# laprade117/interactive-unet

Measured on AMD Instinct MI355X. Metric: voxels/sec (train step + full-volume predict) on 128^3 chunks, higher is better.
Workload: dtype bf16

## Files before the change

interactive-unet_amd/csrc/capi.hip:

```cpp
#include "common.h"
#include <cstdarg>
#include <cstdio>

static thread_local char g_err[512] = "";

void iunet_set_error(const char* fmt, ...) {
  va_list ap;
  va_start(ap, fmt);
  vsnprintf(g_err, sizeof(g_err), fmt, ap);
  va_end(ap);
}

#define DT_OK(dt) IUNET_REQUIRE((dt) == 0 || (dt) == 1, "dtype must be 0 (f16) or 1 (bf16), got %d", (dt))

extern "C" {

const char* iunet_last_error(void) { return g_err; }
int iunet_abi_version(void) { return 1; }

int iunet_conv3_num_tiles(int nd, int N, int D, int H, int W) { return iunet_conv3_tiles(nd, N, D, H, W); }

int iunet_conv3_stats_parts(int nd, int N, int D, int H, int W, int Cout, int layout) {
  return layout >= 2 ? iunet_conv3_v4_stats_parts(nd, Cout) : iunet_conv3_tiles(nd, N, D, H, W);
}

long long iunet_pack_conv3_elems(int Cout, int Cin, int taps, int mode) { return iunet_pack_conv3_size(Cout, Cin, taps, mode); }

int iunet_pack_conv3(int dtype, const void* w, const void* scale, void* dst, int Cout, int Cin, int taps, int mode,
                     void* stream) {
  DT_OK(dtype);
  IUNET_REQUIRE(w && dst, "pack_conv3: null pointer");
  IUNET_REQUIRE(taps == 9 || taps == 27, "pack_conv3: taps must be 9 or 27 (got %d)", taps);
  return iunet_pack_conv3_launch(dtype, (const float*)w, (const float*)scale, dst, Cout, Cin, taps, mode, (hipStream_t)stream);
}

int iunet_pack_first_conv(int dtype, const void* w, const void* scale, void* dst, int Cout, int Cin, int taps,
                          void* stream) {
  DT_OK(dtype);
  IUNET_REQUIRE(w && dst, "pack_first_conv: null pointer");
  IUNET_REQUIRE(Cout % 32 == 0 && Cin >= 1 && Cin <= 12, "pack_first_conv: Cout multiple of 32, Cin 1..4 (3..12: the virtual operator of iunet_x2_prep)");
  return iunet_pack_first_conv_launch(dtype, (const float*)w, (const float*)scale, dst, Cout, Cin, taps, (hipStream_t)stream);
}

long long iunet_pack_first_conv_elems(int Cout, int Cin, int taps) { return (long long)Cout * (((taps * Cin + 31) / 32) * 32); }

int iunet_pack_convT(int dtype, const void* w, void* dst, int Cin, int Cout, int npos, void* stream) {
  DT_OK(dtype);
  IUNET_REQUIRE(w && dst, "pack_convT: null pointer");
  IUNET_REQUIRE(npos == 4 || npos == 8, "pack_convT: npos must be 4 or 8");
  IUNET_REQUIRE(Cin % 32 == 0 && Cout % 32 == 0, "pack_convT: channels must be multiples of 32");
  return iunet_pack_convT_launch(dtype, (const float*)w, dst, Cin, Cout, npos, (hipStream_t)stream);
}

int iunet_conv3_pick_layout(int, int, int, int, int, int, int) { return 2; }

int iunet_conv3_compact_ok(int nd, int N, int D, int H, int W, int Cin, int Cout, int act, int bw) {
  if ((nd != 2 && nd != 3) || N < 1 || D < 1 || H < 1 || W < 1 || Cin < 32 || Cout < 32 || Cin % 32 || Cout % 32 || (bw && nd != 2)) return 0;
  if (nd == 2) return D == 1 && !((act || bw) && Cin > 64);
  if (Cin <= 32) return 0;
  return !(act && Cin > 192);
}

int iunet_conv3_packs_compact(int taps, int Cin) {
  IUNET_REQUIRE(taps == 9 || taps == 27, "conv3_packs_compact: taps must be 9 or 27 (got %d)", taps);
  IUNET_REQUIRE(Cin >= 32 && Cin % 32 == 0, "conv3_packs_compact: Cin must be a positive multiple of 32 (got %d)", Cin);
  return taps == 9 || Cin > 32;
}

int iunet_conv3_plan(int nd, int N, int D, int H, int W, int Cin, int Cout, int act, int bw, int have_compact, int* fused) {
  IUNET_REQUIRE(nd == 2 || nd == 3, "conv3_plan: nd must be 2 or 3 (got %d)", nd);
  IUNET_REQUIRE_GRID("conv3_plan", N, D, H, W);
  IUNET_REQUIRE(Cin >= 32 && Cout >= 32 && Cin % 32 == 0 && Cout % 32 == 0, "conv3_plan: channels must be positive multiples of 32 (%d, %d)", Cin, Cout);
  const int f = (act || bw) && (nd == 3 || Cin <= 64);
  if (fused) *fused = f;
  return have_compact && iunet_conv3_compact_ok(nd, N, D, H, W, Cin, Cout, act && f, bw && f) ? 3 : 2;
}

int iunet_conv3_tile_pairs(int nd, int N, int D, int H, int W, int Cin, int Cout) {
  if ((nd != 2 && nd != 3) || N < 1 || D < 1 || H < 1 || W < 1 || Cin < 32 || Cout < 32 || Cin % 32 || Cout % 32) return 0;
  return iunet_conv3_v4_pairs(nd, N, D, H, W, Cin, Cout, 0);
}

int iunet_conv3_fwd(int dtype, int nd, const void* x, long long x_sstride, void* y, long long y_sstride,
                    const void* wpk, const void* bias, void* stats, int N, int D, int H, int W, int Cin, int Cout,
                    int epi, int layout, void* stream) {
  DT_OK(dtype);
  IUNET_REQUIRE(x && y && wpk, "conv3: null pointer");
  IUNET_REQUIRE(N > 0 && D > 0 && H > 0 && W > 0, "conv3: bad shape %d %d %d %d", N, D, H, W);
  IUNET_REQUIRE(epi >= 0 && epi <= 2, "conv3: bad epilogue %d", epi);
  IUNET_REQUIRE(layout == 2 || layout == 3, "conv3: layout must be 2 or 3 (got %d)", layout);
  return iunet_conv3_launch(dtype, nd, x, x_sstride, y, y_sstride, wpk, (const float*)bias, (float*)stats, N, D, H, W,
                            Cin, Cout, epi, layout, (hipStream_t)stream);
}

int iunet_conv3_fwd_act(int dtype, int nd, const void* x, long long x_sstride, void* y, long long y_sstride,
                        const void* wpk, const void* bias, void* stats, const void* in_scale, const void* in_shift,
                        int N, int D, int H, int W, int Cin, int Cout, int epi, int layout, void* stream) {
  DT_OK(dtype);
  IUNET_REQUIRE(x && y && wpk && in_scale && in_shift, "conv3_act: null pointer");
  IUNET_REQUIRE(N > 0 && D > 0 && H > 0 && W > 0, "conv3: bad shape %d %d %d %d", N, D, H, W);
  IUNET_REQUIRE(epi >= 0 && epi <= 2, "conv3: bad epilogue %d", epi);
  IUNET_REQUIRE(layout == 2 || layout == 3, "conv3_act: the fused input activation exists in layouts 2 and 3 only (got %d)", layout);
  return iunet_conv3_launch(dtype, nd, x, x_sstride, y, y_sstride, wpk, (const float*)bias, (float*)stats, N, D, H, W,
                            Cin, Cout, epi, layout, (hipStream_t)stream, (const float*)in_scale, (const float*)in_shift);
}

int iunet_conv3_sample_stats_rows(int dtype, int nd, int N, int D, int H, int W, int Cin, int Cout, int layout) {
  DT_OK(dtype);
  if (layout < 2 || (nd != 2 && nd != 3) || N < 1 || D < 1 || H < 1 || W < 1 || Cin < 32 || Cout < 32 || Cin % 32 || Cout % 32) return 0;
  if (layout == 3 && !iunet_conv3_compact_ok(nd, N, D, H, W, Cin, Cout, 0, 0)) return 0;
  int rows = 0;
  if (iunet_conv3_v4_launch(dtype, nd, nullptr, 0, nullptr, 0, nullptr, nullptr, nullptr, N, D, H, W, Cin, Cout, 0, nullptr, nullptr, nullptr,
                            nullptr, 0, nullptr, layout == 3, 1, &rows) != IUNET_OK) return 0;
  return rows;
}

int iunet_conv3_fwd_sample_stats(int dtype, int nd, const void* x, long long x_sstride, void* y, long long y_sstride, const void* wpk,
                                 void* stats, int N, int D, int H, int W, int Cin, int Cout, int layout, void* stream) {
  DT_OK(dtype);
  IUNET_REQUIRE(x && y && wpk && stats, "conv3_fwd_sample_stats: null pointer");
  IUNET_REQUIRE_GRID("conv3_fwd_sample_stats", N, D, H, W);
  IUNET_REQUIRE(layout == 2 || layout == 3, "conv3_fwd_sample_stats: layout 2 or 3 (got %d)", layout);
  IUNET_REQUIRE(nd == 2 || nd == 3, "conv3: nd must be 2 or 3 (got %d)", nd);
  IUNET_REQUIRE(nd == 3 || D == 1, "conv3: 2-D conv needs D == 1");
  return iunet_conv3_v4_launch(dtype, nd, x, x_sstride, y, y_sstride, wpk, nullptr, (float*)stats, N, D, H, W, Cin, Cout, 0, nullptr, nullptr,
                               (hipStream_t)stream, nullptr, 0, nullptr, layout == 3, 1, nullptr);
}

int iunet_conv3_dgrad_sample_bnstats(int dtype, int nd, const void* dy, long long dy_sstride, void* dz, long long dz_sstride, const void* wpk,
// ... 209 lines not shown
```

interactive-unet_amd/csrc/conv3_v4.hip:

```cpp
#include "common.h"
#include <cstdlib>
#include <type_traits>

#ifdef IUNET_STAMPS
__device__ unsigned long long g_v4_stamps[4 * 512];
extern "C" int iunet_v4_stamps_read(unsigned long long* out) {
  return (int)hipMemcpyFromSymbol(out, HIP_SYMBOL(g_v4_stamps), sizeof(unsigned long long) * 4 * 512);
}
#endif
__device__ __attribute__((aligned(16))) unsigned int g_v4_zero16[4] = {0u, 0u, 0u, 0u};

namespace {

template <int ND, bool SMALL> struct V4Tile;
template <> struct V4Tile<3, false> { static constexpr int TZ = 4, TY = 8, TX = 16, PADZ = 1, NCOL = 9, S16 = 1, NCW = 8; };
template <> struct V4Tile<3, true>  { static constexpr int TZ = 2, TY = 8, TX = 16, PADZ = 1, NCOL = 9, S16 = 1, NCW = 4; };
template <bool SMALL> struct V4Tile<2, SMALL> { static constexpr int TZ = 1, TY = 16, TX = 32, PADZ = 0, NCOL = 3, S16 = 2, NCW = 8; };

#ifndef V4_BW_LT
#define V4_BW_LT 256
#endif
#ifndef V4_X2_LT3D
#define V4_X2_LT3D 512
#endif
#ifndef V4_RING2
#define V4_RING2 1
#endif
#ifndef V4_NP3_LT
#define V4_NP3_LT 512
#endif
constexpr int v4_loader_threads(int nd, bool ws, bool pair, bool spl, bool bwv = false, bool np = false) { return (ws || pair || ((spl || np) && nd == 2)) ? 256 : bwv ? V4_BW_LT : (spl && nd == 3) ? V4_X2_LT3D : (np && nd == 3) ? V4_NP3_LT : 512; }

struct ConvV4Params {
  const void* x;  long long x_sstride;
  void* y;        long long y_sstride;
  const void* wpk;
  const float* bias;
  const float* in_scale;
  const float* in_shift;
  float* stats;
  int N, D, H, W, Cin, Cout;
  int tilesZ, tilesY, tilesX;
  int bz, by, bx;
  int nbz, nby, nbx;
  int epi;
  int dbg;
  const void* bw_y; long long bw_y_ss;
  const float* bw_mean; const float* bw_invstd; const float* bw_scale; const float* bw_shift;
  int split_nc, x_lo, y_lo;
  const float* oscale;
  int* sat;
  int per_sample;
  int* query_rows;
};

template <typename T, int ND, bool WS, bool SMALL, bool BW = false, bool PAIR = false, bool NP = false, bool SPL = false>
__global__ __launch_bounds__((V4Tile<ND, SMALL>::NCW * 64 + v4_loader_threads(ND, WS, PAIR, SPL, BW, NP)), 1) void conv3_v4_kernel(ConvV4Params p) {
  static_assert(!SPL || (!WS && !BW && !PAIR && !(NP && ND == 3)), "split precision: streamed weights (Cin' = 3 Cin >= 96), forward only, padded operator in 3-D");
  static_assert(!PAIR || (!WS && !BW && ND == 3), "tile pairs: the streamed-weight 3-D forward / data-gradient variant only");
  static_assert(!NP || (!PAIR && (ND == 2 || !WS) && (!BW || (ND == 2 && WS))), "padding-free step: the streamed-weight 3-D variants and the 2-D ones; fused BatchNorm-backward sums on the 2-D resident-weights variant only");
  constexpr bool NP3 = NP && ND == 3, NP2 = NP && ND == 2;
  using V8 = typename Vec8<T>::type;
  using TL = V4Tile<ND, SMALL>;
  constexpr int NCW = TL::NCW, NLT = v4_loader_threads(ND, WS, PAIR, SPL, BW, NP);
  constexpr int TZ = TL::TZ, TY = TL::TY, TX = TL::TX, PADZ = TL::PADZ, NCOL = TL::NCOL, S16 = TL::S16;
  constexpr int FX = TX / 16, NI = TZ * TY * FX / NCW, NR = NI / FX;
  constexpr int PZ = TZ + 2 * PADZ, PY = TY + 2, PX = TX + 2;
  constexpr int NPIX = PZ * PY * PX;
  constexpr int PLANE = ((NPIX * 16 + 255) / 256) * 256;
  constexpr int CP = 2 * S16;
  constexpr int ABUF = CP * PLANE;
  constexpr int NCMB = (NCOL + 1) / 2, KS = NCMB * 3;
  constexpr int WBYTES = KS * 2 * 1024;
  constexpr int WSTEP = NP2 ? 3 * 3 * 2 * 1024 : S16 * WBYTES;
  constexpr bool RING2 = NP2 && !SPL && (WS ? (V4_RING2 & 1) != 0 : (V4_RING2 & 2) != 0);
  constexpr int NBUF = (NP3 || RING2) ? 3 : 2;
  constexpr int OFF_W = NBUF * ABUF;
  constexpr int WE = 4 * 3 * 2 * 1024, WO = WE + 3 * 2 * 1024;
  constexpr int AIT = (NPIX + NLT - 1) / NLT;
  constexpr int WIT = ((NP3 ? WO : WSTEP) / 16 + NLT - 1) / NLT;
  constexpr int NGRP = NP2 ? 3 : S16 * NCMB;
  constexpr int NRD = FX * (NR + 2) + 6;
  static_assert(NCW * NI == TZ * TY * FX, "consumer waves x fragments must cover the tile");

  extern __shared__ __attribute__((aligned(256))) unsigned char smem[];

  const int tid = threadIdx.x, lane = tid & 63;
  const int wave = __builtin_amdgcn_readfirstlane(tid >> 6);
  const int cob = blockIdx.y;
  const int nbricks = p.N * p.nbz * p.nby * p.nbx;
  const int bslots = p.bx * p.by * p.bz, ngrp = (int)gridDim.x / (8 * bslots);
  const int xcd = (blockIdx.x + (nbricks < 8 ? blockIdx.y : 0)) & 7, slot_all = blockIdx.x >> 3;
  const int grp = slot_all / bslots, slot = slot_all - grp * bslots;
  const int sx = slot % p.bx, sy = (slot / p.bx) % p.by, sz = slot / (p.bx * p.by);
  const int xb0 = (int)((long long)xcd * nbricks / 8), xb1 = (int)((long long)(xcd + 1) * nbricks / 8);
  const int b_begin = xb0 + (int)((long long)(xb1 - xb0) * grp / ngrp), b_end = xb0 + (int)((long long)(xb1 - xb0) * (grp + 1) / ngrp);
  const int nchunk = p.Cin / (16 * S16);
  const int nsteps = (b_end - b_begin) * nchunk;
  auto tile_of = [&](int s) -> int { return PAIR ? 2 * (s / (2 * nchunk)) + (s & 1) : s / nchunk; };
// ... 51 lines not shown
    }
    __syncthreads();
  }

  if (wave >= NCW) {
    const unsigned* zero16 = iunet_opaque_ptr((const unsigned*)g_v4_zero16);
    const int lt = tid - NCW * 64;
    int pcoord[AIT];
#pragma unroll
    for (int it = 0; it < AIT; ++it) {
      const int pix = min(lt + it * NLT, NPIX - 1);
      const int px = pix % PX, t2 = pix / PX;
      pcoord[it] = px | ((t2 % PY) << 8) | ((t2 / PY) << 16);
    }
    struct Staged { u32x4 a[AIT][CP]; unsigned ok; };
    const unsigned lds0 = (unsigned)(size_t)(__attribute__((address_space(3))) unsigned char*)smem;
    const int lw = __builtin_amdgcn_readfirstlane(lt >> 6);
    auto dma_weights = [&](int s, int buf, int it0 = 0, int it1 = 1 << 20) {
      const int chunk = chunk_of(s);
      const u32x4* ws = NP3 ? wsrc + (long long)(chunk >> 1) * ((WE + WO) / 16) + ((chunk & 1) ? WE / 16 : 0) : wsrc + (long long)chunk * (WSTEP / 16);
      const int nitem = NP3 ? ((chunk & 1) ? WO / 16 : WE / 16) : WSTEP / 16;
      const int woff = NP3 ? ((chunk & 1) ? WE : 0) : buf * WSTEP;
#pragma unroll
      for (int it = 0; it < WIT; ++it) {
        if (it < it0 || it >= it1) continue;
        const int base = it * NLT + lw * 64;
        if (base < nitem) {
          const u32x4* gsrc = ws + min(base + (lt & 63), nitem - 1);
          const unsigned dst = __builtin_amdgcn_readfirstlane(lds0 + OFF_W + woff + base * 16);
          unsigned keep;
          asm volatile("s_mov_b32 %0, m0\n\ts_mov_b32 m0, %2\n\ts_nop 0\n\tglobal_load_lds_dwordx4 %1, off\n\ts_mov_b32 m0, %0"
                       : "=&s"(keep) : "v"(gsrc), "s"(dst) : "memory");
        }
      }
    };
    auto load = [&](int s, Staged& r) {
      const int chunk = chunk_of(s);
      int n_img, z0, y0, x0;
      tile_origin(tile_of(s), n_img, z0, y0, x0);
      const T* xc = (const T*)p.x + (long long)n_img * p.x_sstride + src_plane(chunk) * plane_stride;
      r.ok = 0;
#pragma unroll
      for (int it = 0; it < AIT; ++it) {
        const int px = pcoord[it] & 255, py = (pcoord[it] >> 8) & 255, pz = pcoord[it] >> 16;
        const int gz = z0 + pz - PADZ, gy = y0 + py - 1, gx = x0 + px - 1;
        const bool ok = (unsigned)gz < (unsigned)p.D && (unsigned)gy < (unsigned)p.H && (unsigned)gx < (unsigned)p.W;
        const int cz = min(max(gz, 0), p.D - 1), cy = min(max(gy, 0), p.H - 1), cx = min(max(gx, 0), p.W - 1);
        const long long goff = (((long long)cz * p.H + cy) * p.W + cx) * 8;
#pragma unroll
        for (int k = 0; k < CP; ++k) r.a[it][k] = *(const u32x4*)(xc + k * plane_stride + goff);
        r.ok |= ok ? (1u << it) : 0u;
      }
    };
    auto dma_acts = [&](int s) {
      const int chunk = chunk_of(s);
      int n_img, z0, y0, x0;
      tile_origin(tile_of(s), n_img, z0, y0, x0);
      const T* xc = (const T*)p.x + (long long)n_img * p.x_sstride + src_plane(chunk) * plane_stride;
      const unsigned abuf = lds0 + abuf_of(s);
#pragma unroll
      for (int it = 0; it < AIT; ++it) {
        const int base = it * NLT + lw * 64;
        if (base < PLANE / 16) {
          const int pix = lt + it * NLT;
          const int px = pcoord[it] & 255, py = (pcoord[it] >> 8) & 255, pz = pcoord[it] >> 16;
          const int gz = z0 + pz - PADZ, gy = y0 + py - 1, gx = x0 + px - 1;
          const bool ok = pix < NPIX && (unsigned)gz < (unsigned)p.D && (unsigned)gy < (unsigned)p.H && (unsigned)gx < (unsigned)p.W;
          const long long goff = (((long long)gz * p.H + gy) * p.W + gx) * 8;
          if (pix < PLANE / 16) {
#pragma unroll
            for (int k = 0; k < CP; ++k) {
              const u32x4* gsrc = ok ? (const u32x4*)(xc + k * plane_stride + goff) : (const u32x4*)zero16;
              const unsigned dst = __builtin_amdgcn_readfirstlane(abuf + k * PLANE + base * 16);
              unsigned keep;
              asm volatile("s_mov_b32 %0, m0\n\ts_mov_b32 m0, %2\n\ts_nop 0\n\tglobal_load_lds_dwordx4 %1, off\n\ts_mov_b32 m0, %0"
                           : "=&s"(keep) : "v"(gsrc), "s"(dst) : "memory");
            }
          }
        }
      }
    };
    auto landed = [&]() { asm volatile("s_waitcnt vmcnt(0)" ::: "memory"); };
    auto commit = [&](int s, const Staged& r, auto ACT) {
      constexpr bool act = decltype(ACT)::value;
      unsigned char* ab = smem + abuf_of(s);
      const int cfirst = chunk_of(s) * CP * 8;
#pragma unroll
      for (int k = 0; k < CP; ++k) {
        float sc[8], sh[8];
        if (act) {
          const f32x4* ap = (const f32x4*)(smem + off_act) + (cfirst + k * 8) / 2;
          const f32x4 s0 = ap[0], s1 = ap[1], h0 = ap[2], h1 = ap[3];
#pragma unroll
          for (int j = 0; j < 4; ++j) { sc[j] = s0[j]; sc[4 + j] = s1[j]; sh[j] = h0[j]; sh[4 + j] = h1[j]; }
        }
#pragma unroll
        for (int it = 0; it < AIT; ++it) {
          const int pix = lt + it * NLT;
          u32x4 v = r.a[it][k];
          asm volatile("" : "+v"(v));
          if (pix < NPIX) {
            const bool ok = (r.ok >> it) & 1u;
            if (act) {
              const V8 in = __builtin_bit_cast(V8, v);
              V8 o;
#pragma unroll
              for (int j = 0; j < 8; ++j) o[j] = from_f32<T>(fmaxf(fmaf(sc[j], to_f32<T>(in[j]), sh[j]), 0.f));
              v = __builtin_bit_cast(u32x4, o);
            }
            *(u32x4*)(ab + k * PLANE + pix * 16) = ok ? v : u32x4{0u, 0u, 0u, 0u};
          }
        }
      }
    };
    auto run = [&](auto ACT) {
      const int last = nsteps - 1;
#ifdef V4_NOLOAD
      lds_barrier();
      for (int s = 0; s < nsteps; ++s) lds_barrier();
      return;
#endif
      if constexpr (RING2) if (!decltype(ACT)::value && !(p.dbg & 64)) {
        int K = 0;
#pragma unroll
        for (int it = 0; it < AIT; ++it) K += (it * NLT + lw * 64 < PLANE / 16) ? CP : 0;
        auto landed_but_last = [&]() {
          if (K == CP * AIT) asm volatile("s_waitcnt vmcnt(%0)" :: "i"(CP * AIT) : "memory");
          else if (K == CP * (AIT - 1)) asm volatile("s_waitcnt vmcnt(%0)" :: "i"(CP * (AIT - 1)) : "memory");
          else landed();
        };
        if (!WS) dma_weights(0, 0);
        dma_acts(0);
        if (last > 0) { dma_acts(1); landed_but_last(); } else landed();
        lds_barrier();
        for (int s = 0; s < nsteps; ++s) {
          if (!WS && s + 1 < nsteps) dma_weights(s + 1, (s + 1) & 1);
          if (s + 2 < nsteps) { dma_acts(s + 2); landed_but_last(); } else landed();
          lds_barrier();
        }
        return;
      }
      if ((ND == 3 || SPL || (NP2 && !WS)) && !decltype(ACT)::value && !(p.dbg & 64)) {
        if (!WS) dma_weights(0, 0);
        dma_acts(0);
        landed();
        lds_barrier();
        if constexpr (SPL) {
          for (int s = 0; s < nsteps; ++s) {
            if (s + 1 < nsteps) {
              const int pn = part_of(s + 1);
              if (pn != 1) dma_weights(s + 1, pn == 2 ? 1 : 0);
              if (pn != 2) dma_acts(s + 1);
            }
            landed();
            lds_barrier();
          }
          return;
        }
        if (PAIR) {
          for (int s = 0; s + 1 < nsteps; s += 2) {
            const bool more = s + 2 < nsteps;
            const int nb = chunk_of(min(s + 2, last)) & 1;
            if (more) dma_weights(s + 2, nb, 0, WIT / 2);
            dma_acts(s + 1);
            landed();
            lds_barrier();
            if (more) { dma_weights(s + 2, nb, WIT / 2, WIT); dma_acts(s + 2); }
            landed();
            lds_barrier();
          }
        } else {
          for (int s = 0; s < nsteps; ++s) {
            if (s + 1 < nsteps) {
              if (!WS) dma_weights(s + 1, (s + 1) & 1);
              dma_acts(s + 1);
            }
            landed();
            lds_barrier();
          }
        }
        return;
      }
      Staged r;
      if (!WS) dma_weights(0, 0);
      load(0, r);
      commit(0, r, ACT);
      load(min(1, last), r);
      if (!WS) asm volatile("s_waitcnt vmcnt(0)" ::: "memory");
      lds_barrier();
      if (WS) {
        for (int s = 0; s < nsteps; ++s) {
          commit(s + 1, r, ACT);
          load(min(s + 2, last), r);
          lds_barrier();
        }
      } else if (PAIR) {
        Staged r2;
        for (int s = 0; s + 1 < nsteps; s += 2) {
          const bool more = s + 2 < nsteps;
          const int nb = chunk_of(min(s + 2, last)) & 1;
          if (more) dma_weights(s + 2, nb, 0, WIT / 2);
          load(min(s + 2, last), r2);
          commit(s + 1, r, ACT);
          lds_barrier();
          if (more) dma_weights(s + 2, nb, WIT / 2, WIT);
          load(min(s + 3, last), r);
          commit(s + 2, r2, ACT);
          lds_barrier();
        }
      } else {
        Staged r2;
        int s = 0;
        for (; s + 1 < nsteps; s += 2) {
          dma_weights(s + 1, 1);
          load(min(s + 2, last), r2);
          commit(s + 1, r, ACT);
          lds_barrier();
          if (!NP3 || s + 2 <= last) dma_weights(min(s + 2, last), 0);
          load(min(s + 3, last), r);
          commit(s + 2, r2, ACT);
          lds_barrier();
        }
        if (s < nsteps) lds_barrier();
      }
    };
    if (p.in_scale != nullptr) run(std::true_type{}); else run(std::false_type{});
    if (p.stats != nullptr) lds_barrier();
    return;
  }

#ifdef V4_PRIO
  if (V4_PRIO >= 2 && wave >= NCW / 2) __builtin_amdgcn_s_setprio(2); else __builtin_amdgcn_s_setprio(1);
// ... 314 lines not shown
  IUNET_REQUIRE(!p.per_sample || (!PAIR && !SPL && nbricks >= 8 && p.stats != nullptr), "conv3 layout 2 / 3: per-sample statistics are not available for this launch (iunet_conv3_sample_stats_rows says 0)");
  if (p.stats != nullptr && !p.per_sample) {
    const int rows = iunet_conv3_v4_stats_parts(ND, p.Cout);
    if (gx < rows)
      IUNET_CHECK_HIP(hipMemsetAsync(p.stats + (long long)gx * p.Cout * 2, 0, (size_t)(rows - gx) * p.Cout * 2 * sizeof(float), stream));
  }
  hipLaunchKernelGGL((conv3_v4_kernel<T, ND, WS, SMALL, BW, PAIR, NP, SPL>), dim3(gx, ncob, nz), dim3(TL::NCW * 64 + v4_loader_threads(ND, WS, PAIR, SPL, BW, NP)), lds, stream, p);
  IUNET_CHECK_HIP(hipGetLastError());
  return IUNET_OK;
}

}

int iunet_conv3_v4_stats_parts(int nd, int Cout) {
  (void)nd;
  const int ncob = Cout / 32;
  return 8 * (ncob == 1 ? 32 : ncob == 2 ? 16 : ncob <= 4 ? 8 : 4);
}

int iunet_conv3_v4_pairs(int nd, int N, int D, int H, int W, int Cin, int Cout, int bw) {
  static const int pair_on = getenv("IUNET_V4_PAIR") ? atoi(getenv("IUNET_V4_PAIR")) : 1;
  if (nd != 3 || bw || !pair_on || Cin <= 32) return 0;
  const int tz = (D + 3) / 4, ty = (H + 7) / 8, tx = (W + 15) / 16;
  if ((long long)N * tz * ty * tx * (Cout / 32) < 128) return 0;
  int bz, by, bx;
  iunet_brick_shape(3, Cout / 32, tz, ty, tx, &bz, &by, &bx);
  const long long nbricks = (long long)N * ((tz + bz - 1) / bz) * ((ty + by - 1) / by) * ((tx + bx - 1) / bx);
  return nbricks % 16 == 0;
}

int iunet_conv3_v4_launch(int dtype, int nd, const void* x, long long x_sstride, void* y, long long y_sstride, const void* wpk,
                          const float* bias, float* stats, int N, int D, int H, int W, int Cin, int Cout, int epi,
                          const float* in_scale, const float* in_shift, hipStream_t stream, const void* bw_y, long long bw_y_ss,
                          const float* const* bw_par, int compact, int per_sample, int* query_rows) {
  IUNET_REQUIRE(Cin % 32 == 0 && Cout % 32 == 0, "conv3 layout 2: Cin %% 32, Cout %% 32 (got %d -> %d)", Cin, Cout);
  ConvV4Params p;
  p.x = x; p.x_sstride = x_sstride; p.y = y; p.y_sstride = y_sstride; p.wpk = wpk; p.bias = bias; p.stats = stats;
  p.N = N; p.D = D; p.H = H; p.W = W; p.Cin = Cin; p.Cout = Cout; p.epi = epi;
  p.in_scale = in_scale; p.in_shift = in_shift;
  p.bw_y = bw_y; p.bw_y_ss = bw_y_ss;
  p.bw_mean = bw_y ? bw_par[0] : nullptr; p.bw_invstd = bw_y ? bw_par[1] : nullptr;
  p.bw_scale = bw_y ? bw_par[2] : nullptr; p.bw_shift = bw_y ? bw_par[3] : nullptr;
  IUNET_REQUIRE(bw_y == nullptr || stats != nullptr, "conv3 layout 2: the fused BatchNorm-backward sums need a statistics buffer");
  p.tilesZ = p.tilesY = p.tilesX = 0;
  p.bz = p.by = p.bx = p.nbz = p.nby = p.nbx = 0;
  p.split_nc = 0; p.x_lo = p.y_lo = 0; p.oscale = nullptr; p.sat = nullptr;
  p.per_sample = per_sample; p.query_rows = query_rows;
#ifdef IUNET_ABLATE
  static const int dbg = getenv("IUNET_V4_DBG") ? atoi(getenv("IUNET_V4_DBG")) : 0;
#else
  static const int dbg = 0;
#endif
  p.dbg = dbg;
  const bool ws = nd == 3 ? Cin <= 32 : Cin <= 64;
  const long long big_tiles = (long long)(per_sample ? 1 : N) * ((D + 3) / 4) * ((H + 7) / 8) * ((W + 15) / 16);
  const bool small = nd == 3 && !ws && big_tiles * (Cout / 32) < 128;
  if (compact) {
    IUNET_REQUIRE((bw_y == nullptr || (nd == 2 && Cin <= 64)) && (nd == 2 || !ws), "conv3 layout 3: fused BatchNorm-backward sums in 2-D up to 64 input channels only; 3-D: Cin > 32");
    if (nd == 2) {
      static const int ws2d = getenv("IUNET_V4_WS2D") ? atoi(getenv("IUNET_V4_WS2D")) : 64;
      const bool ws = (in_scale != nullptr || bw_y != nullptr) ? Cin <= 64 : Cin <= ws2d;
      if (ws && bw_y != nullptr) return dtype == 0 ? launch_v4<f16, 2, true, false, true, false, true>(p, stream) : launch_v4<bf16, 2, true, false, true, false, true>(p, stream);
      if (ws) return dtype == 0 ? launch_v4<f16, 2, true, false, false, false, true>(p, stream) : launch_v4<bf16, 2, true, false, false, false, true>(p, stream);
      return dtype == 0 ? launch_v4<f16, 2, false, false, false, false, true>(p, stream) : launch_v4<bf16, 2, false, false, false, false, true>(p, stream);
    }
    if (small) return dtype == 0 ? launch_v4<f16, 3, false, true, false, false, true>(p, stream) : launch_v4<bf16, 3, false, true, false, false, true>(p, stream);
    return dtype == 0 ? launch_v4<f16, 3, false, false, false, false, true>(p, stream) : launch_v4<bf16, 3, false, false, false, false, true>(p, stream);
  }
  const bool pair = !per_sample && iunet_conv3_v4_pairs(nd, N, D, H, W, Cin, Cout, bw_y != nullptr) != 0;
  if (pair) return dtype == 0 ? launch_v4<f16, 3, false, false, false, true>(p, stream) : launch_v4<bf16, 3, false, false, false, true>(p, stream);
#define V4_GO(TT, BWV) (nd == 3 ? (ws ? launch_v4<TT, 3, true, false, BWV>(p, stream)                                          \
                                      : (small ? launch_v4<TT, 3, false, true, BWV>(p, stream) : launch_v4<TT, 3, false, false, BWV>(p, stream))) \
                                : (ws ? launch_v4<TT, 2, true, false, BWV>(p, stream) : launch_v4<TT, 2, false, false, BWV>(p, stream)))
  if (bw_y != nullptr) return dtype == 0 ? V4_GO(f16, true) : V4_GO(bf16, true);
  return dtype == 0 ? V4_GO(f16, false) : V4_GO(bf16, false);
#undef V4_GO
}

int iunet_conv3_v4_x2_pack_mode(int nd) {
  static const int np2 = getenv("IUNET_X2_NP2") ? atoi(getenv("IUNET_X2_NP2")) : 1;
  return nd == 2 && np2 ? 6 : 2;
}

int iunet_conv3_v4_x2_launch(int nd, const void* x, long long x_sstride, int x_lo, void* y, long long y_sstride, int y_lo, const void* wpk,
                             const float* oscale, const float* bias, int N, int D, int H, int W, int Cin, int Cout, int epi,
                             int* sat, hipStream_t stream) {
  IUNET_REQUIRE(Cin % 32 == 0 && Cout % 32 == 0, "conv3 x2: Cin %% 32, Cout %% 32 (got %d -> %d)", Cin, Cout);
  ConvV4Params p;
  p.x = x; p.x_sstride = x_sstride; p.y = y; p.y_sstride = y_sstride; p.wpk = wpk; p.bias = bias; p.stats = nullptr;
  p.N = N; p.D = D; p.H = H; p.W = W; p.Cin = 3 * Cin; p.Cout = Cout; p.epi = epi;
  p.in_scale = p.in_shift = nullptr;
  p.bw_y = nullptr; p.bw_y_ss = 0; p.bw_mean = p.bw_invstd = p.bw_scale = p.bw_shift = nullptr;
  p.tilesZ = p.tilesY = p.tilesX = 0;
  p.bz = p.by = p.bx = p.nbz = p.nby = p.nbx = 0;
  p.dbg = 0;
  p.split_nc = Cin / (nd == 3 ? 16 : 32); p.x_lo = x_lo; p.y_lo = y_lo; p.oscale = oscale; p.sat = sat;
  p.per_sample = 0; p.query_rows = nullptr;
  if (nd == 2) {
    if (iunet_conv3_v4_x2_pack_mode(2) == 6) return launch_v4<f16, 2, false, false, false, false, true, true>(p, stream);
    return launch_v4<f16, 2, false, false, false, false, false, true>(p, stream);
  }
  const long long big_tiles = (long long)N * ((D + 3) / 4) * ((H + 7) / 8) * ((W + 15) / 16);
  const bool small = big_tiles * (Cout / 32) < 128;
  return small ? launch_v4<f16, 3, false, true, false, false, false, true>(p, stream)
               : launch_v4<f16, 3, false, false, false, false, false, true>(p, stream);
}
```

interactive-unet_amd/csrc/conv3_wgrad_v2.hip:

```cpp
#include "common.h"
#include <cstdlib>
#include <type_traits>

#ifdef IUNET_STAMPS
__device__ unsigned long long g_wg2_stamps[4 * 512];
extern "C" int iunet_wg2_stamps_read(unsigned long long* out) {
  return (int)hipMemcpyFromSymbol(out, HIP_SYMBOL(g_wg2_stamps), sizeof(unsigned long long) * 4 * 512);
}
#endif
__device__ __attribute__((aligned(16))) unsigned int g_wg2_zero16[4] = {0u, 0u, 0u, 0u};

namespace {

typedef short s16x4 __attribute__((ext_vector_type(4)));
typedef short s16x8 __attribute__((ext_vector_type(8)));
typedef __attribute__((address_space(3))) s16x4* lds_s4_ptr;

struct WgradV2Params {
  const void* x;  long long x_ss;
  const void* dy; long long dy_ss;
  const float* x_scale;
  const float* x_shift;
  float* slab;
  int N, D, H, W, Cin, Cout;
  int tilesZ, tilesY, tilesX;
  int dbg;
};

template <typename T>
__device__ __forceinline__ typename Vec8<T>::type tr_frag_v2(unsigned addr) {
  const s16x4 lo = __builtin_amdgcn_ds_read_tr16_b64_v4i16((lds_s4_ptr)addr);
  const s16x4 hi = __builtin_amdgcn_ds_read_tr16_b64_v4i16((lds_s4_ptr)(addr + 64));
  const s16x8 v = __builtin_shufflevector(lo, hi, 0, 1, 2, 3, 4, 5, 6, 7);
  return __builtin_bit_cast(typename Vec8<T>::type, v);
}

template <typename T, bool DYR>
__global__ __launch_bounds__(768, 1) void conv3_wgrad_v2_kernel(WgradV2Params p) {
  constexpr int TZ = 2, TY = 8, TX = 16, TAPS = 27;
  constexpr int PY = TY + 2, PX = TX + 2;
  constexpr int ZPIX = PY * PX;
  constexpr int NSLOT = 6;
  constexpr int NVOX = TZ * TY * TX;
  constexpr int NKS = NVOX / 32;
  constexpr int PLANE_X = NSLOT * ZPIX * 16 + 192;
  constexpr int PLANE_Y = ((NVOX * 16 + 255) / 256) * 256 + 64;
  constexpr int OFF_Y = 4 * PLANE_X;
  constexpr int YBUF = 4 * PLANE_Y;
  constexpr int NCW = 8, NLT = 256;
  constexpr int NU = TAPS * 2, MAXU = (NU + NCW - 1) / NCW;
  constexpr int XIT = (4 * ZPIX + 63) / 64;
  constexpr int YIT = NVOX * 4 / NLT;
  static_assert(PLANE_X % 256 == 64, "x plane stride must be 64 mod 256");

  extern __shared__ __attribute__((aligned(256))) unsigned char smem[];
  const unsigned lds0 = (unsigned)(size_t)(__attribute__((address_space(3))) unsigned char*)smem;

  const int tid = threadIdx.x, lane = tid & 63;
  const int wave = __builtin_amdgcn_readfirstlane(tid >> 6);
  const int cob = blockIdx.y, cib = blockIdx.z;
  const int tiles_per_sample = p.tilesZ * p.tilesY * p.tilesX;
  const int ntiles = tiles_per_sample * p.N;
  const long long plane_stride = (long long)p.D * p.H * p.W * 8;
  const int lb = xcd_remap(blockIdx.x, gridDim.x);
  const int t_begin = (int)((long long)lb * ntiles / gridDim.x), t_end = (int)((long long)(lb + 1) * ntiles / gridDim.x);
  const int nt = t_end - t_begin;

  auto tile_origin = [&](int k, int& n_img, int& z0, int& y0, int& x0) {
    const int tile = t_begin + k;
    n_img = tile / tiles_per_sample;
    int trem = tile - n_img * tiles_per_sample;
    const int tz_i = trem % p.tilesZ; trem /= p.tilesZ;
    const int tx_i = trem % p.tilesX, ty_i = trem / p.tilesX;
    z0 = tz_i * TZ; y0 = ty_i * TY; x0 = tx_i * TX;
  };
  auto fresh = [&](int k) { return k == 0 || (t_begin + k) % p.tilesZ == 0; };

  if (wave >= NCW) {
    const unsigned* zero16 = iunet_opaque_ptr((const unsigned*)g_wg2_zero16);
    const int lt = tid - NCW * 64;
    if (p.x_scale == nullptr && !(p.dbg & 4)) {
      const int lw = __builtin_amdgcn_readfirstlane(lt >> 6), ll = lt & 63;
      int xcd[3], ycd[4];
#pragma unroll
      for (int j = 0; j < 3; ++j) {
        const int pix = j * 64 + ll;
        xcd[j] = pix < ZPIX ? ((pix / PX) << 8) | (pix % PX) : -1;
      }
#pragma unroll
      for (int j = 0; j < 4; ++j) {
        const int pix = j * 64 + ll;
        ycd[j] = (pix % TX) | (((pix / TX) % TY) << 8) | ((pix / (TX * TY)) << 16);
      }
      auto dma16 = [&](const void* gsrc, unsigned dst) {
        unsigned keep;
        asm volatile("s_mov_b32 %0, m0\n\ts_mov_b32 m0, %2\n\ts_nop 0\n\tglobal_load_lds_dwordx4 %1, off\n\ts_mov_b32 m0, %0"
                     : "=&s"(keep) : "v"(gsrc), "s"(dst) : "memory");
      };
      auto dma_x = [&](int k, int pz_lo, int pz_hi, int slot_first) {
        int n_img, z0, y0, x0;
        tile_origin(k, n_img, z0, y0, x0);
        const T* xin = (const T*)p.x + (long long)n_img * p.x_ss + (long long)(cib * 4 + lw) * plane_stride;
        for (int pz = pz_lo; pz < pz_hi; ++pz) {
          const int slot = (slot_first + pz - pz_lo) % NSLOT;
          const int gz = z0 + pz - 1;
#pragma unroll
          for (int j = 0; j < 3; ++j) {
            if (xcd[j] >= 0) {
              const int gy = y0 + (xcd[j] >> 8) - 1, gx = x0 + (xcd[j] & 255) - 1;
              const bool ok = (unsigned)gz < (unsigned)p.D && (unsigned)gy < (unsigned)p.H && (unsigned)gx < (unsigned)p.W;
              const void* gsrc = ok ? (const void*)(xin + (((long long)gz * p.H + gy) * p.W + gx) * 8) : (const void*)zero16;
              dma16(gsrc, __builtin_amdgcn_readfirstlane(lds0 + lw * PLANE_X + slot * (ZPIX * 16) + j * 1024));
            }
          }
        }
      };
      auto dma_y = [&](int k) {
        int n_img, z0, y0, x0;
        tile_origin(k, n_img, z0, y0, x0);
        const T* dyin = (const T*)p.dy + (long long)n_img * p.dy_ss + (long long)(cob * 4 + lw) * plane_stride;
#pragma unroll
        for (int j = 0; j < 4; ++j) {
          const int gz = z0 + (ycd[j] >> 16), gy = y0 + ((ycd[j] >> 8) & 255), gx = x0 + (ycd[j] & 255);
          const bool ok = gz < p.D && gy < p.H && gx < p.W;
          const void* gsrc = ok ? (const void*)(dyin + (((long long)gz * p.H + gy) * p.W + gx) * 8) : (const void*)zero16;
          dma16(gsrc, __builtin_amdgcn_readfirstlane(lds0 + OFF_Y + (k & 1) * YBUF + lw * PLANE_Y + j * 1024));
        }
      };
      auto landed = [&]() { asm volatile("s_waitcnt vmcnt(0)" ::: "memory"); };
      const bool refill = !(p.dbg & 1);
      int base = 0;
      if (nt > 0) { dma_x(0, 0, 4, 0); dma_y(0); }
      landed();
      lds_barrier();
      for (int k = 0; k < nt; ++k) {
        const bool more = k + 1 < nt && refill;
        const bool fr = more && fresh(k + 1);
        if (more) {
          if (fr) dma_x(k + 1, 0, 2, base + 4); else dma_x(k + 1, 2, 4, base + 4);
          dma_y(k + 1);
        }
        landed();
        lds_barrier();
        if (k + 1 < nt && fresh(k + 1)) {
          if (fr) dma_x(k + 1, 2, 4, base + 6);
          landed();
          lds_barrier();
          base = (base + 4) % NSLOT;
        } else {
          base = (base + 2) % NSLOT;
        }
      }
      return;
    }
    struct Staged { u32x4 x[XIT]; u32x4 y[YIT]; unsigned okx, oky; };
    const int lw = lt >> 6, ll = lt & 63;
    int xc[XIT], xl[XIT], yc[YIT], yl[YIT];
#pragma unroll
    for (int it = 0; it < XIT; ++it) {
      const int idx = min(ll + it * 64, 4 * ZPIX - 1);
      const int zi = idx / ZPIX, pix = idx - zi * ZPIX;
      const int py = pix / PX, px = pix - py * PX;
      xc[it] = zi | (py << 8) | (px << 16);
      xl[it] = lw * PLANE_X + pix * 16;
    }
    float xsc[8], xsh[8];
#pragma unroll
    for (int j = 0; j < 8; ++j) {
      xsc[j] = p.x_scale ? p.x_scale[cib * 32 + lw * 8 + j] : 1.f;
      xsh[j] = p.x_scale ? p.x_shift[cib * 32 + lw * 8 + j] : 0.f;
    }
#pragma unroll
    for (int it = 0; it < YIT; ++it) {
      const int item = lt + it * NLT;
      const int pl = item / NVOX, pix = item - pl * NVOX;
      const int px = pix % TX, t2 = pix / TX, py = t2 % TY, pz = t2 / TY;
      yc[it] = pz | (pl << 4) | (py << 8) | (px << 16);
      yl[it] = pl * PLANE_Y + pix * 16;
    }
    auto load = [&](int k, Staged& r) {
      int n_img, z0, y0, x0;
      tile_origin(k, n_img, z0, y0, x0);
      const bool fr = fresh(k);
      const int nitems = (fr ? 4 : 2) * ZPIX, pz0 = fr ? 0 : 2;
      const T* xin = (const T*)p.x + (long long)n_img * p.x_ss + (long long)(cib * 4 + lw) * plane_stride;
      const T* dyin = (const T*)p.dy + (long long)n_img * p.dy_ss + (long long)cob * 4 * plane_stride;
      r.okx = 0; r.oky = 0;
#pragma unroll
      for (int it = 0; it < XIT; ++it) {
        if (ll + it * 64 < nitems) {
          const int zi = xc[it] & 15, py = (xc[it] >> 8) & 255, px = xc[it] >> 16;
          const int gz = z0 + pz0 + zi - 1, gy = y0 + py - 1, gx = x0 + px - 1;
          const bool ok = (unsigned)gz < (unsigned)p.D && (unsigned)gy < (unsigned)p.H && (unsigned)gx < (unsigned)p.W;
          const int cz = min(max(gz, 0), p.D - 1), cy = min(max(gy, 0), p.H - 1), cx = min(max(gx, 0), p.W - 1);
          r.x[it] = *(const u32x4*)(xin + (long long)((cz * p.H + cy) * p.W + cx) * 8);
          r.okx |= ok ? (1u << it) : 0u;
        }
      }
#pragma unroll
// ... 210 lines not shown
    if (k + 1 < nt && fresh(k + 1)) {
      lds_barrier();
      base = (base + 4) % NSLOT;
    } else {
      base = (base + 2) % NSLOT;
    }
  }

#ifdef IUNET_STAMPS
  if (wave == 0 && lane == 0 && cob == 0 && cib == 0 && blockIdx.x < 512) {
    const unsigned long long st1 = __builtin_amdgcn_s_memtime(), sr1 = __builtin_amdgcn_s_memrealtime();
    g_wg2_stamps[blockIdx.x * 4 + 0] = st1 - st0; g_wg2_stamps[blockIdx.x * 4 + 1] = sr1 - sr0; g_wg2_stamps[blockIdx.x * 4 + 2] = nt;
  }
#endif
  const int ncob = gridDim.y, ncib = gridDim.z;
  float* slab = p.slab + ((((long long)blockIdx.x * ncob + cob) * ncib + cib) * TAPS) * 1024;
#pragma unroll
  for (int i = 0; i < MAXU; ++i) {
    const int u = uw + NCW * i;
    if (u < NU) {
      const int tap = u >> 1, cih = u & 1;
#pragma unroll
      for (int t = 0; t < 2; ++t)
#pragma unroll
        for (int j = 0; j < 4; ++j) slab[tap * 1024 + (t * 16 + 4 * g + j) * 32 + cih * 16 + i16] = acc[i][t][j];
    }
  }
}

}

int iunet_conv3_wgrad_v2_blocks(int N, int D, int H, int W, int Cin, int Cout) {
  const long long ntiles = (long long)N * ((D + 1) / 2) * ((H + 7) / 8) * ((W + 15) / 16);
  const int pairs = (Cin / 32) * (Cout / 32);
  long long nb = (256 + pairs - 1) / pairs;
  if (nb > ntiles) nb = ntiles;
  if (nb < 1) nb = 1;
  return (int)nb;
}

int iunet_conv3_wgrad_v2_launch(int dtype, const void* x, long long x_ss, const void* dy, long long dy_ss, float* slab,
                                int N, int D, int H, int W, int Cin, int Cout, const float* x_scale, const float* x_shift,
                                hipStream_t stream) {
  WgradV2Params p;
  p.x = x; p.x_ss = x_ss; p.dy = dy; p.dy_ss = dy_ss; p.slab = slab; p.x_scale = x_scale; p.x_shift = x_shift;
  p.N = N; p.D = D; p.H = H; p.W = W; p.Cin = Cin; p.Cout = Cout;
  p.tilesZ = (D + 1) / 2; p.tilesY = (H + 7) / 8; p.tilesX = (W + 15) / 16;
#ifdef IUNET_ABLATE
  static const int dbg = getenv("IUNET_WG2_DBG") ? atoi(getenv("IUNET_WG2_DBG")) : 0;
#else
  static const int dbg = 0;
#endif
  p.dbg = dbg;
  static const int dyr = getenv("IUNET_WG2_DYR") ? atoi(getenv("IUNET_WG2_DYR")) : 1;
  constexpr int PLANE_X = 6 * 180 * 16 + 192, PLANE_Y = 256 * 16 + 64;
  constexpr int LDS = 4 * PLANE_X + 2 * 4 * PLANE_Y;
  const int nb = iunet_conv3_wgrad_v2_blocks(N, D, H, W, Cin, Cout);
  dim3 grid(nb, Cout / 32, Cin / 32);
  if (dtype == 0) {
    if (dyr) { IUNET_SET_MAX_LDS((conv3_wgrad_v2_kernel<f16, true>), LDS); hipLaunchKernelGGL((conv3_wgrad_v2_kernel<f16, true>), grid, dim3(768), LDS, stream, p); }
    else { IUNET_SET_MAX_LDS((conv3_wgrad_v2_kernel<f16, false>), LDS); hipLaunchKernelGGL((conv3_wgrad_v2_kernel<f16, false>), grid, dim3(768), LDS, stream, p); }
  } else {
    if (dyr) { IUNET_SET_MAX_LDS((conv3_wgrad_v2_kernel<bf16, true>), LDS); hipLaunchKernelGGL((conv3_wgrad_v2_kernel<bf16, true>), grid, dim3(768), LDS, stream, p); }
    else { IUNET_SET_MAX_LDS((conv3_wgrad_v2_kernel<bf16, false>), LDS); hipLaunchKernelGGL((conv3_wgrad_v2_kernel<bf16, false>), grid, dim3(768), LDS, stream, p); }
  }
  IUNET_CHECK_HIP(hipGetLastError());
  return IUNET_OK;
}
```

interactive-unet_amd/csrc/launchers.h:

```cpp
#pragma once
#include <hip/hip_runtime.h>

void iunet_set_error(const char* fmt, ...);

int iunet_conv3_launch(int dtype, int nd, const void* x, long long x_sstride, void* y, long long y_sstride,
                       const void* wpk, const float* bias, float* stats, int N, int D, int H, int W, int Cin,
                       int Cout, int epi, int layout, hipStream_t stream, const float* in_scale = nullptr,
                       const float* in_shift = nullptr, const void* bw_y = nullptr, long long bw_y_ss = 0,
                       const float* const* bw_par = nullptr);
int iunet_conv3_tiles(int nd, int N, int D, int H, int W);
long long iunet_pack_conv3_size(int Cout, int Cin, int taps, int mode);
int iunet_pack_conv3_launch(int dtype, const float* w, const float* scale, void* dst, int Cout, int Cin, int taps,
                            int mode, hipStream_t stream);

int iunet_conv3_v4_launch(int dtype, int nd, const void* x, long long x_sstride, void* y, long long y_sstride, const void* wpk,
                          const float* bias, float* stats, int N, int D, int H, int W, int Cin, int Cout, int epi,
                          const float* in_scale, const float* in_shift, hipStream_t stream, const void* bw_y = nullptr,
                          long long bw_y_ss = 0, const float* const* bw_par = nullptr, int compact = 0, int per_sample = 0,
                          int* query_rows = nullptr);
int iunet_conv3_v4_stats_parts(int nd, int Cout);
int iunet_conv3_v4_pairs(int nd, int N, int D, int H, int W, int Cin, int Cout, int bw);
int iunet_conv3_v4_x2_launch(int nd, const void* x, long long x_sstride, int x_lo, void* y, long long y_sstride, int y_lo, const void* wpk,
                             const float* oscale, const float* bias, int N, int D, int H, int W, int Cin, int Cout, int epi,
                             int* sat, hipStream_t stream);
int iunet_conv3_v4_x2_pack_mode(int nd);

int iunet_first_conv_launch(int dtype, int nd, const void* x, int in_dtype, long long sN, long long sC, long long sD,
                            long long sH, long long sW, void* y, long long y_sstride, const void* w,
                            const float* bias, float* stats, int N, int D, int H, int W, int Cin, int Cout, int relu,
                            hipStream_t stream, int out8 = 0);
int iunet_pack_first_conv_launch(int dtype, const float* w, const float* scale, void* dst, int Cout, int Cin, int taps,
                                 hipStream_t stream);
int iunet_maxpool_launch(int dtype, int nd, const void* x, long long x_ss, void* y, long long y_ss, int planes, int N,
                         int Do, int Ho, int Wo, hipStream_t stream);
int iunet_maxpool_q_launch(int nd, const void* x, long long x_ss, void* y, long long y_ss, int planes16, int N, int Do, int Ho, int Wo,
                           hipStream_t stream);
int iunet_convT_launch(int dtype, int nd, const void* x, long long x_ss, void* y, long long y_ss, const void* wpk,
                       const float* bias, int N, int D, int H, int W, int Cin, int Cout, hipStream_t stream, int out8 = 0);
int iunet_pack_convT_launch(int dtype, const float* w, void* dst, int Cin, int Cout, int npos, hipStream_t stream);
int iunet_head_launch(int dtype, const void* x, long long x_ss, int C0, const float* w, const float* bias, int ncls,
                      float* logits, float* probs, unsigned char* cls, const long long* os, float divisor, int accumulate, int N,
                      int D, int H, int W,
                      hipStream_t stream);

long long iunet_f32_pack_size(int Cout, int Cin, int taps);
int iunet_f32_pack_launch(const float* w, float* dst, float* bias_out, const float* gamma, const float* beta,
                          const float* mean, const float* var, float eps, int Cout, int Cin, int taps, int transposed,
                          hipStream_t stream);
int iunet_f32_conv_launch(int nd, const void* x, int in_dtype, const long long* st, float* y, long long y_ss, const float* wpk,
                          const float* bias, int N, int D, int H, int W, int Cin, int Cout, int relu, int transposed,
                          hipStream_t stream);
int iunet_f32_maxpool_launch(int nd, const float* x, long long x_ss, float* y, long long y_ss, int C, int N, int Do, int Ho,
                             int Wo, hipStream_t stream);
int iunet_f32_head_launch(const float* x, long long x_ss, int C0, const float* w, const float* bias, int ncls, float* logits,
                          float* probs, unsigned char* cls, const long long* os, float divisor, int accumulate, int N, int D,
                          int H, int W, hipStream_t stream);

long long iunet_f8_pack_bytes(int Cout, int Cin, int taps);
int iunet_f8_pack_launch(const float* w, const float* gamma, const float* beta, const float* mean, const float* var, float eps,
                         void* dst, float* wscale, float* bias_out, int Cout, int Cin, int taps, hipStream_t stream);
long long iunet_conv3_f8_workspace_floats(int nd, int N, int D, int H, int W, int Cin, int Cout);
int iunet_conv3_f8_launch(int dtype, int nd, const void* x, long long x_sstride, void* y, long long y_sstride, const void* wpk,
                          const float* wscale, const float* bias, int N, int D, int H, int W, int Cin, int Cout, int epi,
                          float* workspace, hipStream_t stream);
int iunet_conv3_f8_launch_q(int dtype, int nd, const void* x, long long x_sstride, int x_fmt, void* y, long long y_sstride, int y_fmt,
                            const void* wpk, const float* wscale, const float* bias, int N, int D, int H, int W, int Cin, int Cout,
                            int epi, float* workspace, hipStream_t stream);

int iunet_f8_k128(int taps, int Cin);
int iunet_conv3_f8k_launch(int dtype, const void* x, long long x_sstride, void* y, long long y_sstride, const void* wpk,
                           const float* wscale, const float* bias, int N, int D, int H, int W, int Cin, int Cout, int epi,
                           int ksplit, float* partial, int small, int in8, int out8, hipStream_t stream);

int iunet_conv3_wgrad_v2_blocks(int N, int D, int H, int W, int Cin, int Cout);
// ... 10 lines not shown
```

Baseline: 686.9 million.

## DMA raw activations into LDS and apply BN+ReLU in place for fused-act convs

When the input needs a fused BatchNorm scale/shift plus ReLU, the loader waves now copy raw activations straight into LDS with the direct DMA path and then apply the affine+ReLU in place. Previously such inputs went through register staging and commit. The weight-gradient kernel gets the same treatment for its x operand. An env switch chooses the mode: by default forward uses it only when IUNET_ACT_DMA >= 2 for 3-D or >= 3 for 2-D, while wgrad uses it for 3-D. The change trades staging registers for an extra LDS read-modify-write and serialized waits.

```diff
diff --git a/interactive-unet_amd/csrc/capi.hip b/interactive-unet_amd/csrc/capi.hip
--- a/interactive-unet_amd/csrc/capi.hip
+++ b/interactive-unet_amd/csrc/capi.hip
@@ -75,6 +75,16 @@
   if (fused) *fused = f;
   return have_compact && iunet_conv3_compact_ok(nd, N, D, H, W, Cin, Cout, act && f, bw && f) ? 3 : 2;
 }
+
+}
+int iunet_conv3_act_dma(int kind, int nd, int Cin) {
+  static const int mode = getenv("IUNET_ACT_DMA") ? atoi(getenv("IUNET_ACT_DMA")) : 1;
+  (void)Cin;
+  if (mode <= 0) return 0;
+  if (kind == 0) return mode >= (nd == 3 ? 2 : 3);
+  return nd == 3;
+}
+extern "C" {
 
 int iunet_conv3_tile_pairs(int nd, int N, int D, int H, int W, int Cin, int Cout) {
   if ((nd != 2 && nd != 3) || N < 1 || D < 1 || H < 1 || W < 1 || Cin < 32 || Cout < 32 || Cin % 32 || Cout % 32) return 0;
diff --git a/interactive-unet_amd/csrc/conv3_v4.hip b/interactive-unet_amd/csrc/conv3_v4.hip
--- a/interactive-unet_amd/csrc/conv3_v4.hip
+++ b/interactive-unet_amd/csrc/conv3_v4.hip
@@ -45,6 +45,7 @@
   int nbz, nby, nbx;
   int epi;
   int dbg;
+  int act_dma;
   const void* bw_y; long long bw_y_ss;
   const float* bw_mean; const float* bw_invstd; const float* bw_scale; const float* bw_shift;
   int split_nc, x_lo, y_lo;
@@ -202,12 +203,13 @@
         r.ok |= ok ? (1u << it) : 0u;
       }
     };
-    auto dma_acts = [&](int s) {
+    auto dma_acts = [&](int s) -> unsigned {
       const int chunk = chunk_of(s);
       int n_img, z0, y0, x0;
       tile_origin(tile_of(s), n_img, z0, y0, x0);
       const T* xc = (const T*)p.x + (long long)n_img * p.x_sstride + src_plane(chunk) * plane_stride;
       const unsigned abuf = lds0 + abuf_of(s);
+      unsigned okm = 0;
 #pragma unroll
       for (int it = 0; it < AIT; ++it) {
         const int base = it * NLT + lw * 64;
@@ -216,6 +218,7 @@
           const int px = pcoord[it] & 255, py = (pcoord[it] >> 8) & 255, pz = pcoord[it] >> 16;
           const int gz = z0 + pz - PADZ, gy = y0 + py - 1, gx = x0 + px - 1;
           const bool ok = pix < NPIX && (unsigned)gz < (unsigned)p.D && (unsigned)gy < (unsigned)p.H && (unsigned)gx < (unsigned)p.W;
+          okm |= ok ? (1u << it) : 0u;
           const long long goff = (((long long)gz * p.H + gy) * p.W + gx) * 8;
           if (pix < PLANE / 16) {
 #pragma unroll
@@ -229,8 +232,38 @@
           }
         }
       }
+      return okm;
     };
     auto landed = [&]() { asm volatile("s_waitcnt vmcnt(0)" ::: "memory"); };
+    auto activate_in_lds = [&](int s, unsigned okm) {
+      unsigned char* ab = smem + abuf_of(s);
+      const int cfirst = chunk_of(s) * CP * 8;
+      u32x4 v[AIT][CP];
+#pragma unroll
+      for (int it = 0; it < AIT; ++it) {
+        const int pixc = min(lt + it * NLT, NPIX - 1);
+#pragma unroll
+        for (int k = 0; k < CP; ++k) v[it][k] = *(const u32x4*)(ab + k * PLANE + pixc * 16);
+      }
+#pragma unroll
+      for (int k = 0; k < CP; ++k) {
+        float sc[8], sh[8];
+        const f32x4* ap = (const f32x4*)(smem + off_act) + (cfirst + k * 8) / 2;
+        const f32x4 s0 = ap[0], s1 = ap[1], h0 = ap[2], h1 = ap[3];
+#pragma unroll
+        for (int j = 0; j < 4; ++j) { sc[j] = s0[j]; sc[4 + j] = s1[j]; sh[j] = h0[j]; sh[4 + j] = h1[j]; }
+#pragma unroll
+        for (int it = 0; it < AIT; ++it) {
+          if ((okm >> it) & 1u) {
+            const V8 in = __builtin_bit_cast(V8, v[it][k]);
+            V8 o;
+#pragma unroll
+            for (int j = 0; j < 8; ++j) o[j] = from_f32<T>(fmaxf(fmaf(sc[j], to_f32<T>(in[j]), sh[j]), 0.f));
+            *(u32x4*)(ab + k * PLANE + (lt + it * NLT) * 16) = __builtin_bit_cast(u32x4, o);
+          }
+        }
+      }
+    };
     auto commit = [&](int s, const Staged& r, auto ACT) {
       constexpr bool act = decltype(ACT)::value;
       unsigned char* ab = smem + abuf_of(s);
@@ -328,6 +361,23 @@
             landed();
             lds_barrier();
           }
+        }
+        return;
+      }
+      if constexpr (decltype(ACT)::value && !PAIR && !SPL) if (p.act_dma) {
+        if (!WS) dma_weights(0, 0);
+        unsigned okm = dma_acts(0);
+        landed();
+        activate_in_lds(0, okm);
+        lds_barrier();
+        for (int s = 0; s < nsteps; ++s) {
+          if (s + 1 < nsteps) {
+            if (!WS) dma_weights(s + 1, (s + 1) & 1);
+            okm = dma_acts(s + 1);
+            landed();
+            activate_in_lds(s + 1, okm);
+          }
+          lds_barrier();
         }
         return;
       }
@@ -748,6 +798,7 @@
   static const int dbg = 0;
 #endif
   p.dbg = dbg;
+  p.act_dma = in_scale != nullptr && iunet_conv3_act_dma(0, nd, Cin) != 0;
   const bool ws = nd == 3 ? Cin <= 32 : Cin <= 64;
   const long long big_tiles = (long long)(per_sample ? 1 : N) * ((D + 3) / 4) * ((H + 7) / 8) * ((W + 15) / 16);
   const bool small = nd == 3 && !ws && big_tiles * (Cout / 32) < 128;
@@ -789,7 +840,7 @@
   p.bw_y = nullptr; p.bw_y_ss = 0; p.bw_mean = p.bw_invstd = p.bw_scale = p.bw_shift = nullptr;
   p.tilesZ = p.tilesY = p.tilesX = 0;
   p.bz = p.by = p.bx = p.nbz = p.nby = p.nbx = 0;
-  p.dbg = 0;
+  p.dbg = 0; p.act_dma = 0;
   p.split_nc = Cin / (nd == 3 ? 16 : 32); p.x_lo = x_lo; p.y_lo = y_lo; p.oscale = oscale; p.sat = sat;
   p.per_sample = 0; p.query_rows = nullptr;
   if (nd == 2) {
diff --git a/interactive-unet_amd/csrc/conv3_wgrad_v2.hip b/interactive-unet_amd/csrc/conv3_wgrad_v2.hip
--- a/interactive-unet_amd/csrc/conv3_wgrad_v2.hip
+++ b/interactive-unet_amd/csrc/conv3_wgrad_v2.hip
@@ -25,6 +25,7 @@
   int N, D, H, W, Cin, Cout;
   int tilesZ, tilesY, tilesX;
   int dbg;
+  int act_dma;
 };
 
 template <typename T>
@@ -79,7 +80,7 @@
   if (wave >= NCW) {
     const unsigned* zero16 = iunet_opaque_ptr((const unsigned*)g_wg2_zero16);
     const int lt = tid - NCW * 64;
-    if (p.x_scale == nullptr && !(p.dbg & 4)) {
+    if ((p.x_scale == nullptr || p.act_dma) && !(p.dbg & 4)) {
       const int lw = __builtin_amdgcn_readfirstlane(lt >> 6), ll = lt & 63;
       int xcd[3], ycd[4];
 #pragma unroll
@@ -128,10 +129,48 @@
         }
       };
       auto landed = [&]() { asm volatile("s_waitcnt vmcnt(0)" ::: "memory"); };
+      const bool actx = p.x_scale != nullptr;
+      float xsc[8], xsh[8];
+#pragma unroll
+      for (int j = 0; j < 8; ++j) {
+        xsc[j] = actx ? p.x_scale[cib * 32 + lw * 8 + j] : 1.f;
+        xsh[j] = actx ? p.x_shift[cib * 32 + lw * 8 + j] : 0.f;
+      }
+      auto act_x = [&](int k, int pz_lo, int pz_hi, int slot_first) {
+        if (!actx) return;
+        int n_img, z0, y0, x0;
+        tile_origin(k, n_img, z0, y0, x0);
+        for (int pz = pz_lo; pz < pz_hi; pz += 2) {
+          u32x4 v[2][3];
+          unsigned char* at[2];
+#pragma unroll
+          for (int h = 0; h < 2; ++h) {
+            at[h] = smem + lw * PLANE_X + ((slot_first + pz + h - pz_lo) % NSLOT) * (ZPIX * 16) + ll * 16;
+#pragma unroll
+            for (int j = 0; j < 3; ++j) v[h][j] = *(const u32x4*)(at[h] + (xcd[j] >= 0 ? j * 1024 : 0));
+          }
+#pragma unroll
+          for (int h = 0; h < 2; ++h) {
+            const int gz = z0 + pz + h - 1;
+#pragma unroll
+            for (int j = 0; j < 3; ++j) {
+              const int gy = y0 + (xcd[j] >> 8) - 1, gx = x0 + (xcd[j] & 255) - 1;
+              if (xcd[j] >= 0 && (unsigned)gz < (unsigned)p.D && (unsigned)gy < (unsigned)p.H && (unsigned)gx < (unsigned)p.W) {
+                const typename Vec8<T>::type in = __builtin_bit_cast(typename Vec8<T>::type, v[h][j]);
+                typename Vec8<T>::type o;
+#pragma unroll
+                for (int c = 0; c < 8; ++c) o[c] = from_f32<T>(fmaxf(fmaf(xsc[c], to_f32<T>(in[c]), xsh[c]), 0.f));
+                *(u32x4*)(at[h] + j * 1024) = __builtin_bit_cast(u32x4, o);
+              }
+            }
+          }
+        }
+      };
       const bool refill = !(p.dbg & 1);
       int base = 0;
       if (nt > 0) { dma_x(0, 0, 4, 0); dma_y(0); }
       landed();
+      if (nt > 0) act_x(0, 0, 4, 0);
       lds_barrier();
       for (int k = 0; k < nt; ++k) {
         const bool more = k + 1 < nt && refill;
@@ -141,10 +180,12 @@
           dma_y(k + 1);
         }
         landed();
+        if (more) { if (fr) act_x(k + 1, 0, 2, base + 4); else act_x(k + 1, 2, 4, base + 4); }
         lds_barrier();
         if (k + 1 < nt && fresh(k + 1)) {
           if (fr) dma_x(k + 1, 2, 4, base + 6);
           landed();
+          if (fr) act_x(k + 1, 2, 4, base + 6);
           lds_barrier();
           base = (base + 4) % NSLOT;
         } else {
@@ -461,6 +502,7 @@
   static const int dbg = 0;
 #endif
   p.dbg = dbg;
+  p.act_dma = x_scale != nullptr && iunet_conv3_act_dma(1, 3, Cin) != 0;
   static const int dyr = getenv("IUNET_WG2_DYR") ? atoi(getenv("IUNET_WG2_DYR")) : 1;
   constexpr int PLANE_X = 6 * 180 * 16 + 192, PLANE_Y = 256 * 16 + 64;
   constexpr int LDS = 4 * PLANE_X + 2 * 4 * PLANE_Y;
diff --git a/interactive-unet_amd/csrc/launchers.h b/interactive-unet_amd/csrc/launchers.h
--- a/interactive-unet_amd/csrc/launchers.h
+++ b/interactive-unet_amd/csrc/launchers.h
@@ -20,6 +20,7 @@
                           int* query_rows = nullptr);
 int iunet_conv3_v4_stats_parts(int nd, int Cout);
 int iunet_conv3_v4_pairs(int nd, int N, int D, int H, int W, int Cin, int Cout, int bw);
+int iunet_conv3_act_dma(int kind, int nd, int Cin);
 int iunet_conv3_v4_x2_launch(int nd, const void* x, long long x_sstride, int x_lo, void* y, long long y_sstride, int y_lo, const void* wpk,
                              const float* oscale, const float* bias, int N, int D, int H, int W, int Cin, int Cout, int epi,
                              int* sat, hipStream_t stream);
```

Result: no change. 688.5 million (median of 5 runs) (+0.2%).
